# GestaltCogTeam/STEP

Hardware: AMD Instinct MI355X
Metric: training windows/sec on PEMS04, horizon-12 MAE parity, 1/2/4/8 MI355X (higher is better)
Workload: dtype f16 (TSFormer Q/K/weights) + bf16 (P, V, GraphWaveNet / graph-learner GEMMs) operands, f32 accumulate

## Files before the change

### include/step_hip.h

```cpp
#ifndef STEP_HIP_H
#define STEP_HIP_H

#include <stdint.h>

#ifdef __cplusplus
extern "C" {
#endif

const char* step_last_error(void);
int step_abi_version(void);

typedef struct StepGemm {
    int M, N, K, batch;
    const void* A; long sam, sak, sab; int a_bf16;
    const void* B; long sbk, sbn, sbb; int b_bf16;
    float* C; long ldc, scn, scb;
    float alpha;
    int accumulate;
    const float* bias; int relu;
    int splitk;
    int a_kblk; long a_kstride;
    int b_kblk; long b_kstride;
    int b_nblk; long b_nstride;
    int c_nblk; long c_nstride;
// ... 8 lines not shown
int step_gemm(const StepGemm* g, void* stream);

#define STEP_ENC_F16 1
#define STEP_ENC_ALWAYS_RESHIFT 2
#define STEP_ENC_RANGE_FLAG 4
#define STEP_ENC_WORKGROUPS(n) (((n) & 0xffff) << 8)
int step_tsformer_encode(const float* series, int S, int L, const void* wpack, long wpack_bytes,
                         int depth, int flags, uint16_t* hidden_bf16, float* hidden_f32, float* last_f32,
                         float* sqnorm_part, float dropout_p, const uint64_t* drop_pool, long pool_words, uint64_t seed,
                         unsigned int* fallback_count, void* stream);
int step_dropout_pool_fill(uint64_t* pool, long words, float dropout_p, uint64_t seed, void* stream);
long step_tsformer_dropout_words(int L, int depth);

int step_pack_long_history(const float* x, int B, int L, int N, int C, int ch, float* out, void* stream);
int step_gather_windows(const float* data, int T, int N, int C, int ch, const long* t0, int B, int L, int H,
                        float* long_series, float* hist, float* fut, void* stream);

long step_knn_workspace_bytes(int B, int N, int F);
int step_knn_graph(const uint16_t* hidden, const float* sqnorm_part, int B, int N, int F, int k_total,
                   float* sim, float* adj, void* work, long work_bytes, void* stream);
int step_topk_mask(const float* sim, int B, int N, int k_total, float* adj, void* work, long work_bytes,
                   void* stream);

typedef struct StepDglParams {
    float *conv1_w, *conv1_b;
    float *conv2_w, *conv2_b;
    float *fc_w, *fc_b;
    float *bn1_w, *bn1_b, *bn1_rm, *bn1_rv;
    float *bn2_w, *bn2_b, *bn2_rm, *bn2_rv;
    float *bn3_w, *bn3_b, *bn3_rm, *bn3_rv;
    float *fc_out_w, *fc_out_b;
    float *fc_cat_w, *fc_cat_b;
    int gemm_bf16;
} StepDglParams;

long step_dgl_global_saved_floats(int N, int T);
long step_dgl_global_work_floats(int N, int T, int backward);
int step_dgl_global_forward(const float* series_nt, int N, int T, const StepDglParams* p, int training,
                            float momentum, float* saved, float* work, float* g, void* stream);
int step_dgl_global_backward(const float* series_nt, int N, int T, const StepDglParams* p, const float* saved,
                             const float* dg, float* work, const StepDglParams* grads, void* stream);
#define STEP_DGL_FRESH_FC_GRAD 16
int step_dgl_global_backward_phase(const float* series_nt, int N, int T, const StepDglParams* p, const float* saved,
                             const float* dg, float* work, const StepDglParams* grads, int phase, void* stream);

typedef struct StepDglShard { int own1; double count1, count2; } StepDglShard;
int step_dgl_global_forward_shard(const float* series_slice, int N, int Ts, const StepDglParams* p, int training, float momentum,
                                  float* saved, float* work, double* sums, float* g, const StepDglShard* shard, int phase,
                                  void* stream);
int step_dgl_global_backward_shard(const float* series_slice, int N, int Ts, const StepDglParams* p, const float* saved,
                                   const float* dg, float* work, const StepDglParams* grads, const StepDglShard* shard, int phase,
                                   void* stream);
long step_dgl_global_offset(int N, int T, int item);

long step_dgl_edges_saved_floats(int B, int N);
long step_dgl_edges_work_floats(int N);
long step_dgl_edges_theta_offset(int N);
int step_dgl_edges_forward(const float* g, int N, int B, const StepDglParams* p, const float* u, uint64_t seed,
                           float temperature, float* saved, float* theta_out, float* adj_out, void* stream);
int step_dgl_edges_backward(const float* g, int N, int B, const StepDglParams* p, const float* saved,
                            const float* dtheta, const float* dadj, float temperature, float* work,
                            const StepDglParams* grads, float* dg, void* aux_stream, void* stream);

typedef struct StepGwnetParams {
    float *nodevec1, *nodevec2;
    float *start_w, *start_b;
    float *filter_w[8], *filter_b[8];
    float *gate_w[8], *gate_b[8];
    float *skip_w[8], *skip_b[8];
    float *bn_w[8], *bn_b[8], *bn_rm[8], *bn_rv[8];
    float *gconv_w[8], *gconv_b[8];
    float *fc_his0_w, *fc_his0_b, *fc_his2_w, *fc_his2_b;
    float *end1_w, *end1_b, *end2_w, *end2_b;
    int gemm_bf16;
} StepGwnetParams;

long step_gwnet_saved_floats(int B, int N, int dropout);
long step_gwnet_work_floats(int B, int N, int backward);
long step_gwnet_saved_offset(int B, int N, int dropout, int item, int layer);
int step_gwnet_forward(const float* hist, int B, int N, int Cin, const float* hidden_last, const float* adj,
                       const StepGwnetParams* p, int training, float dropout_p, uint64_t seed, float momentum,
                       float* saved, float* work, float* pred, void* stream);
int step_gwnet_forward_phase(const float* hist, int B, int N, int Cin, const float* hidden_last, const float* adj,
                             const StepGwnetParams* p, int training, float dropout_p, uint64_t seed, float momentum,
                             float* saved, float* work, float* pred, int phase, void* stream);
int step_gwnet_backward(const float* hist, int B, int N, int Cin, const float* hidden_last, const StepGwnetParams* p,
                        const float* saved, float* work, const float* dpred, const StepGwnetParams* grads,
                        float* dadj, int dropout, void* aux_stream, void* leaf_stream, void* stream);

int step_pt_dropout(const float* x, float* y, long n, float p, uint64_t seed, uint32_t site, void* stream);
int step_pt_ffn_hidden_fwd(const float* x, const float* w1, const float* b1, long R, float p, uint64_t seed, uint32_t site,
                           uint16_t* hidden, void* stream);
int step_pt_ffn_hidden_bwd(const float* dy, const float* w2, const uint16_t* hidden, long R, float p, uint16_t* dhidden, void* stream);
int step_pt_colsum_bf16(const uint16_t* x, long rows, int cols, float* out, void* stream);
long step_pt_rows_linear_pack_bytes(int nkc, int nog);
int step_pt_rows_linear_pack(const float* w, long swo, long swi, int nkc, int nog, const float* bias, void* pack, void* stream);
int step_pt_rows_linear(const void* x, int x_bf16, long R, const void* pack, int nkc, int nog, void* y, int y_bf16, int accumulate, void* stream);
int step_pt_layer_pack(const float* wi, const float* bi, const float* wo, const float* bo, const float* w1, const float* b1, const float* w2,
                       const float* b2, void* ffn, void* qkv, void* o, void* da, void* dx, void* stream);
long step_pt_proj_wgrad_ws_floats(long R);
int step_pt_proj_wgrad(const float* x, const uint16_t* dqkv, const float* dov, const uint16_t* a, long R, float* ws, float* dwi, float* dbi, float* dwo,
                       void* stream);
int step_pt_ffn_fused_fwd_ln(const float* h1, long R, const void* pack, float p, const uint64_t* pool, long pool_words, uint64_t seed, uint32_t site_hidden,
                             uint32_t site_out, const float* gamma, const float* beta, float* pre, float* y, float* stats, void* stream);
int step_pt_rows_linear_ln(const uint16_t* x, long R, const void* pack, const float* res, float p, uint64_t seed, uint32_t site, const float* gamma,
                           const float* beta, float* pre, float* y, float* stats, void* stream);
// ... 123 lines not shown
```

### step_amd/_lib.py

```python
import ctypes
import os

import torch

_HERE = os.path.dirname(os.path.abspath(__file__))
LIB_PATH = os.environ.get("STEP_HIP_LIB") or os.path.join(_HERE, "libstep_hip.so")

_vp, _i, _l, _f, _u64 = ctypes.c_void_p, ctypes.c_int, ctypes.c_long, ctypes.c_float, ctypes.c_uint64


class StepGemm(ctypes.Structure):
    _fields_ = [("M", _i), ("N", _i), ("K", _i), ("batch", _i),
                ("A", _vp), ("sam", _l), ("sak", _l), ("sab", _l), ("a_bf16", _i),
                ("B", _vp), ("sbk", _l), ("sbn", _l), ("sbb", _l), ("b_bf16", _i),
                ("C", _vp), ("ldc", _l), ("scn", _l), ("scb", _l),
                ("alpha", _f), ("accumulate", _i), ("bias", _vp), ("relu", _i), ("splitk", _i),
                ("a_kblk", _i), ("a_kstride", _l), ("b_kblk", _i), ("b_kstride", _l),
                ("b_nblk", _i), ("b_nstride", _l), ("c_nblk", _i), ("c_nstride", _l),
                ("a_kscale", _vp), ("a_kshift", _vp), ("a_kperiod", _i),
                ("batch0", _i), ("sab1", _l), ("sbb1", _l), ("scb1", _l), ("compute_bf16", _i), ("a_rowsum", _vp), ("c_nscale", _vp), ("c_nshift", _vp), ("c_mvec", _vp),
                ("c_nperiod", _i), ("splitk_ws", _vp), ("splitk_ws_floats", _l)]


class StepDglParams(ctypes.Structure):
    NAMES = ["conv1_w", "conv1_b", "conv2_w", "conv2_b", "fc_w", "fc_b",
             "bn1_w", "bn1_b", "bn1_rm", "bn1_rv", "bn2_w", "bn2_b", "bn2_rm", "bn2_rv",
             "bn3_w", "bn3_b", "bn3_rm", "bn3_rv", "fc_out_w", "fc_out_b", "fc_cat_w", "fc_cat_b"]
    _fields_ = [(n, _vp) for n in NAMES] + [("gemm_bf16", _i)]


class StepGwnetParams(ctypes.Structure):
    _fields_ = [("nodevec1", _vp), ("nodevec2", _vp), ("start_w", _vp), ("start_b", _vp),
                ("filter_w", _vp * 8), ("filter_b", _vp * 8), ("gate_w", _vp * 8), ("gate_b", _vp * 8),
                ("skip_w", _vp * 8), ("skip_b", _vp * 8),
                ("bn_w", _vp * 8), ("bn_b", _vp * 8), ("bn_rm", _vp * 8), ("bn_rv", _vp * 8),
                ("gconv_w", _vp * 8), ("gconv_b", _vp * 8),
                ("fc_his0_w", _vp), ("fc_his0_b", _vp), ("fc_his2_w", _vp), ("fc_his2_b", _vp),
                ("end1_w", _vp), ("end1_b", _vp), ("end2_w", _vp), ("end2_b", _vp), ("gemm_bf16", _i)]


_PD = ctypes.POINTER(StepDglParams)


class StepDynState(ctypes.Structure):
    _fields_ = [("seed_xor", ctypes.c_uint64), ("adam_step", ctypes.c_int32), ("lr", _f), ("gsl_coef", _f), ("reserved", _f)]


class StepDglShard(ctypes.Structure):
    _fields_ = [("own1", ctypes.c_int), ("count1", ctypes.c_double), ("count2", ctypes.c_double)]


_PS = ctypes.POINTER(StepDglShard)
_PG = ctypes.POINTER(StepGwnetParams)

_SIGS = {
    "step_last_error": (ctypes.c_char_p, []),
    "step_abi_version": (_i, []),
    "step_gemm": (_i, [ctypes.POINTER(StepGemm), _vp]),
    "step_tsformer_encode": (_i, [_vp, _i, _i, _vp, _l, _i, _i, _vp, _vp, _vp, _vp, _f, _vp, _l, _u64, _vp, _vp]),
    "step_dropout_pool_fill": (_i, [_vp, _l, _f, _u64, _vp]),
    "step_tsformer_dropout_words": (_l, [_i, _i]),
    "step_gather_windows": (_i, [_vp, _i, _i, _i, _i, _vp, _i, _i, _i, _vp, _vp, _vp, _vp]),
    "step_pack_long_history": (_i, [_vp, _i, _i, _i, _i, _i, _vp, _vp]),
    "step_knn_workspace_bytes": (_l, [_i, _i, _i]),
    "step_knn_graph": (_i, [_vp, _vp, _i, _i, _i, _i, _vp, _vp, _vp, _l, _vp]),
    "step_topk_mask": (_i, [_vp, _i, _i, _i, _vp, _vp, _l, _vp]),
    "step_selftest_mfma": (_i, [_vp, _vp]),
    "step_streams_concurrent": (_i, [_vp, _vp, ctypes.POINTER(_i)]),
    "step_dgl_global_saved_floats": (_l, [_i, _i]),
    "step_dgl_global_work_floats": (_l, [_i, _i, _i]),
    "step_dgl_global_forward": (_i, [_vp, _i, _i, _PD, _i, _f, _vp, _vp, _vp, _vp]),
    "step_dgl_global_backward": (_i, [_vp, _i, _i, _PD, _vp, _vp, _vp, _PD, _vp]),
    "step_dgl_global_backward_phase": (_i, [_vp, _i, _i, _PD, _vp, _vp, _vp, _PD, _i, _vp]),
    "step_dgl_global_forward_shard": (_i, [_vp, _i, _i, _PD, _i, _f, _vp, _vp, _vp, _vp, _PS, _i, _vp]),
    "step_dgl_global_backward_shard": (_i, [_vp, _i, _i, _PD, _vp, _vp, _vp, _PD, _PS, _i, _vp]),
    "step_dgl_global_offset": (_l, [_i, _i, _i]),
    "step_dgl_edges_saved_floats": (_l, [_i, _i]),
    "step_dgl_edges_work_floats": (_l, [_i]),
    "step_dgl_edges_theta_offset": (_l, [_i]),
    "step_dgl_edges_forward": (_i, [_vp, _i, _i, _PD, _vp, _u64, _f, _vp, _vp, _vp, _vp]),
    "step_dgl_edges_backward": (_i, [_vp, _i, _i, _PD, _vp, _vp, _vp, _f, _vp, _PD, _vp, _vp, _vp]),
    "step_gwnet_saved_floats": (_l, [_i, _i, _i]),
    "step_gwnet_work_floats": (_l, [_i, _i, _i]),
    "step_gwnet_saved_offset": (_l, [_i, _i, _i, _i, _i]),
    "step_gwnet_forward": (_i, [_vp, _i, _i, _i, _vp, _vp, _PG, _i, _f, _u64, _f, _vp, _vp, _vp, _vp]),
    "step_gwnet_forward_phase": (_i, [_vp, _i, _i, _i, _vp, _vp, _PG, _i, _f, _u64, _f, _vp, _vp, _vp, _i, _vp]),
    "step_gwnet_backward": (_i, [_vp, _i, _i, _i, _vp, _PG, _vp, _vp, _vp, _PG, _vp, _i, _vp, _vp, _vp]),
    "step_pt_dropout": (_i, [_vp, _vp, _l, _f, _u64, ctypes.c_uint32, _vp]),
    "step_pt_ffn_hidden_fwd": (_i, [_vp, _vp, _vp, _l, _f, _u64, ctypes.c_uint32, _vp, _vp]),
    "step_pt_ffn_hidden_bwd": (_i, [_vp, _vp, _vp, _l, _f, _vp, _vp]),
    "step_pt_colsum_bf16": (_i, [_vp, _l, _i, _vp, _vp]),
    "step_pt_rows_linear_pack_bytes": (_l, [_i, _i]),
    "step_pt_rows_linear_pack": (_i, [_vp, _l, _l, _i, _i, _vp, _vp, _vp]),
    "step_pt_rows_linear": (_i, [_vp, _i, _l, _vp, _i, _i, _vp, _i, _i, _vp]),
    "step_pt_layer_pack": (_i, [_vp] * 14),
    "step_pt_proj_wgrad_ws_floats": (_l, [_l]),
    "step_pt_proj_wgrad": (_i, [_vp, _vp, _vp, _vp, _l, _vp, _vp, _vp, _vp, _vp]),
    "step_pt_ffn_fused_fwd_ln": (_i, [_vp, _l, _vp, _f, _vp, _l, _u64, ctypes.c_uint32, ctypes.c_uint32, _vp, _vp, _vp, _vp, _vp, _vp]),
    "step_pt_rows_linear_ln": (_i, [_vp, _l, _vp, _vp, _f, _u64, ctypes.c_uint32, _vp, _vp, _vp, _vp, _vp, _vp]),
    "step_pt_embed_unmasked_fwd": (_i, [_vp, _vp, _vp, _vp, _vp, _l, _i, _i, _f, _u64, ctypes.c_uint32, _vp, _vp]),
    "step_pt_embed_unmasked_bwd": (_i, [_vp, _vp, _vp, _l, _i, _i, _f, _u64, ctypes.c_uint32, _vp, _vp, _vp, _vp]),
    "step_pt_dec_input_bwd_sums": (_i, [_vp, _l, _i, _i, _f, _u64, ctypes.c_uint32, _vp, _vp, _vp, _vp, _vp]),
    "step_pt_ffn_pack_bytes": (_l, []),
    "step_pt_ffn_wgrad_workgroups": (_l, [_l]),
    "step_pt_ffn_wgrad_ws_floats": (_l, [_l]),
    "step_pt_ffn_pack": (_i, [_vp, _vp, _vp, _vp, _vp, _vp]),
    "step_pt_ffn_fused_fwd": (_i, [_vp, _l, _vp, _f, _vp, _l, _u64, ctypes.c_uint32, _vp, _vp]),
    "step_pt_ffn_fused_bwd_data": (_i, [_vp, _vp, _l, _vp, _f, _vp, _l, _u64, ctypes.c_uint32, _vp, _vp]),
    "step_pt_ffn_fused_bwd_weights": (_i, [_vp, _vp, _l, _vp, _vp, _f, _vp, _l, _u64, ctypes.c_uint32, _vp, _vp, _vp, _vp, _vp]),
    "step_pt_add_layernorm_fwd": (_i, [_vp, _vp, _l, _f, _u64, ctypes.c_uint32, _vp, _vp, _vp, _vp, _vp, _vp]),
    "step_pt_layernorm_bwd_dropout": (_i, [_vp, _vp, _l, _vp, _vp, _vp, _vp, _f, _u64, ctypes.c_uint32, _vp, _vp, _vp, _vp]),
    "step_pt_dropout_relu_mask": (_i, [_vp, _vp, _l, _f, _u64, ctypes.c_uint32, _vp]),
    "step_pt_add_dropout": (_i, [_vp, _vp, _vp, _l, _f, _u64, ctypes.c_uint32, _vp]),
    "step_pt_add_rows": (_i, [_vp, _l, _i, _vp, _vp, _vp]),
    "step_pt_sum_over_seq": (_i, [_vp, _l, _i, _i, _i, _vp, _vp, _vp]),
    "step_pt_token_gather": (_i, [_vp, _l, _i, _vp, _i, _f, _vp, _vp]),
    "step_pt_token_scatter": (_i, [_vp, _l, _i, _vp, _i, _f, _vp, _vp]),
    "step_pt_dec_input": (_i, [_vp, _vp, _vp, _vp, _l, _i, _i, _f, _u64, ctypes.c_uint32, _vp, _vp]),
    "step_pt_dec_input_bwd": (_i, [_vp, _l, _i, _i, _f, _u64, ctypes.c_uint32, _vp, _vp, _vp]),
    "step_pt_layernorm_fwd": (_i, [_vp, _l, _vp, _vp, _vp, _vp, _vp]),
    "step_pt_layernorm_bwd": (_i, [_vp, _vp, _l, _vp, _vp, _vp, _vp, _vp, _vp]),
    "step_pt_attention_fwd": (_i, [_vp, _l, _i, _f, _u64, ctypes.c_uint32, _vp, _vp, _vp]),
    "step_pt_attention_bwd": (_i, [_vp, _vp, _vp, _vp, _l, _i, _f, _u64, ctypes.c_uint32, _vp, _vp]),
    "step_pt_attention_fwd_bf16": (_i, [_vp, _l, _i, _f, _u64, ctypes.c_uint32, _vp, _vp, _vp, _vp, _l, _vp]),
    "step_pt_attention_bwd_bf16": (_i, [_vp, _vp, _vp, _vp, _l, _i, _f, _u64, ctypes.c_uint32, _vp, _vp, _vp]),
    "step_pt_linear_bf16out": (_i, [_vp, _vp, _l, _l, _vp, _l, _i, _i, _vp, _vp]),
    "step_pt_relu_mask": (_i, [_vp, _vp, _l, _vp]),
    "step_colsum": (_i, [_vp, _l, _i, _l, _vp, _vp]),
    "step_loss_fwd_bwd": (_i, [_vp, _vp, _l, _vp, _vp, _l, _f, _f, _vp, _vp, _vp, _vp, _vp]),
# ... 115 lines not shown
```

### step_amd/build.py

```python
import os
import subprocess
import sys

HERE = os.path.dirname(os.path.abspath(__file__))
CSRC = os.path.join(HERE, "csrc")
LIB = os.path.join(HERE, "libstep_hip.so")
SOURCES = ["errors.cpp", "comm.cpp", "gemm.hip", "gemm_bf16.hip", "tsformer_encoder.hip", "knn.hip", "selftest.hip",
           "dgl.hip", "dgl_conv_mfma.hip", "gwnet.hip", "optim.hip", "pretrain.hip", "pretrain_fused.hip", "pretrain_attn2.hip",
           "eval_cache.hip", "eval_metrics.hip", "train_tail.hip"]


def _newer(target, deps):
    if not os.path.exists(target):
        return True
    t = os.path.getmtime(target)
    return any(os.path.getmtime(d) > t for d in deps)


def build(force=False, verbose=True):
    hipcc = os.environ.get("HIPCC", "/opt/rocm/bin/hipcc")
    srcs = [os.path.join(CSRC, s) for s in SOURCES if os.path.exists(os.path.join(CSRC, s))]
    hdrs = [os.path.join(CSRC, f) for f in os.listdir(CSRC) if f.endswith(".h")]
    hdrs.append(os.path.join(HERE, "..", "include", "step_hip.h"))
    objs = []
    os.makedirs(os.path.join(HERE, "build"), exist_ok=True)
    procs = []
    for s in srcs:
        o = os.path.join(HERE, "build", os.path.basename(s) + ".o")
        objs.append(o)
        if force or _newer(o, [s] + hdrs):
            cmd = [hipcc, "--offload-arch=gfx950", "-O3", "-std=c++17", "-fPIC", "-x", "hip", "-c", s, "-o", o]
            if verbose:
                print(" ".join(cmd), flush=True)
            procs.append((s, subprocess.Popen(cmd, stdout=subprocess.PIPE, stderr=subprocess.STDOUT)))
    for s, p in procs:
        out, _ = p.communicate()
        if p.returncode != 0:
            sys.stderr.write(out.decode())
            raise RuntimeError("hipcc failed on " + s)
    if force or _newer(LIB, objs):
        cmd = [hipcc, "--offload-arch=gfx950", "-shared", "-fPIC", "-o", LIB] + objs + ["-ldl"]
        if verbose:
            print(" ".join(cmd), flush=True)
        subprocess.check_call(cmd)
    return LIB


if __name__ == "__main__":
    build(force="--force" in sys.argv)
```

### step_amd/csrc/dgl.hip

```cpp
#include "common.h"
#include "step_internal.h"

namespace {

constexpr int KW = 10;
constexpr int EMB = 100;

template <int CI, int CO, int TPT>
__global__ __launch_bounds__(256) void conv_relu_fwd_kernel(const float* __restrict__ in, const float* __restrict__ w,
                                                            const float* __restrict__ b, const float* __restrict__ in_sc,
                                                            const float* __restrict__ in_sh, float* __restrict__ out,
                                                            float* __restrict__ partial, int Tin, int stat_limit) {
    __shared__ __attribute__((aligned(16))) float ws[CI * KW * CO];
    __shared__ float red[4][2 * CO];
    const int tid = threadIdx.x, n = blockIdx.y;
    const int Tout = Tin - (KW - 1);
    for (int e = tid; e < CI * KW * CO; e += 256) {
        int co = e % CO, k = (e / CO) % KW, ci = e / (CO * KW);
        ws[e] = w[(co * CI + ci) * KW + k];
    }
    __syncthreads();
    const int t0 = (blockIdx.x * 256 + tid) * TPT;
    float acc[CO][TPT];
#pragma unroll
// ... 622 lines not shown
    __shared__ float red[4][32];
    const int o = blockIdx.y, t = blockIdx.x * 256 + threadIdx.x, tid = threadIdx.x;
    const float cso = colsum[o];
    float d[32];
#pragma unroll
    for (int i = 0; i < 32; ++i) d[i] = 0.f;
    if (t < T2) {
        const float4* src = (const float4*)(graw + ((long)o * T2 + t) * 16);
        const float4 g0 = src[0], g1 = src[1], g2 = src[2], g3 = src[3];
        const float g[16] = {g0.x, g0.y, g0.z, g0.w, g1.x, g1.y, g1.z, g1.w, g2.x, g2.y, g2.z, g2.w, g3.x, g3.y, g3.z, g3.w};
        float w[16], old[16];
#pragma unroll
        for (int c = 0; c < 16; ++c) { const long idx = ((long)o * 16 + c) * T2 + t; w[c] = fc_w[idx]; old[c] = overwrite ? 0.f : dfc_w[idx]; }
#pragma unroll
        for (int c = 0; c < 16; ++c) {
            dfc_w[((long)o * 16 + c) * T2 + t] = old[c] + st2[c] * g[c] + st2[16 + c] * cso;
            d[2 * c] = w[c] * g[c]; d[2 * c + 1] = w[c] * cso;
        }
    }
#pragma unroll
    for (int i = 0; i < 32; ++i) {
        const float v = wave_sum(d[i]);
        if ((tid & 63) == 0) red[tid >> 6][i] = v;
    }
    __syncthreads();
    if (tid < 32) atomicAdd(&dots_o[o * 32 + tid], red[0][tid] + red[1][tid] + red[2][tid] + red[3][tid]);
}
__global__ void dots_reduce_kernel(const float* __restrict__ dots_o, float* __restrict__ dots) {
    const int i = threadIdx.x;
    if (i >= 32) return;
    double a = 0.0;
    for (int o = 0; o < EMB; ++o) a += dots_o[o * 32 + i];
    dots[i] = (float)a;
}

static bool dgl_channels_last(const StepDglParams* p) {
    const char* e = getenv("STEP_DGL_F32_STORAGE");
    return p->gemm_bf16 && !(e && e[0] == '1');
}

static bool dgl_legacy_bn_backward() {
    const char* e = getenv("STEP_DGL_LEGACY_BN");
    return e && e[0] == '1';
}

extern "C" long step_dgl_global_saved_floats(int N, int T) {
    long T1 = T - 9, T2 = T - 18;
    return (long)N * 8 * T1 + (long)N * 16 * T2 + (long)N * EMB + 4 * 8 + 4 * 16 + 4 * EMB + (long)EMB * 16 * T2 + 128;
}
static long fc_splitk_ws_floats(int N, int T2) {
    const int splits = step_gemm_auto_splitk(N, EMB, 16 * T2, 1);
    return splits > 1 ? (long)splits * N * EMB + 4 : 0;
}
extern "C" long step_dgl_global_work_floats(int N, int T, int backward) {
    long T1 = T - 9, T2 = T - 18;
    long nb1 = (long)N * cdiv(T1, 1024), nb2 = (long)N * cdiv(T2, 1024);
    long part = (nb1 > nb2 ? nb1 : nb2) * 32 + 64;
    if (!backward) return part + dgl_conv2_pack_floats() + 64 + fc_splitk_ws_floats(N, (int)T2);
    return part + (long)N * 16 * T2 + (long)N * 8 * T1 + (long)EMB * 16 * T2 + 2L * N * EMB + DGL_SMALL + dgl_conv2_wgrad_scratch_floats(N, (int)T1);
}

static float* saved_wp(float* saved, int N, int T) {
    long T1 = T - 9, T2 = T - 18;
    return saved + (long)N * 8 * T1 + (long)N * 16 * T2 + (long)N * EMB + 4 * 8 + 4 * 16 + 4 * EMB;
}
static void carve_saved(float* saved, int N, int T, float** a1, float** a2, float** gpre, float** st1, float** st2, float** st3) {
    long T1 = T - 9, T2 = T - 18;
    *a1 = saved; saved += (long)N * 8 * T1;
    *a2 = saved; saved += (long)N * 16 * T2;
    *gpre = saved; saved += (long)N * EMB;
    *st1 = saved; saved += 4 * 8;
    *st2 = saved; saved += 4 * 16;
    *st3 = saved;
}

static int dgl_bn_stats(const float* partial, int nblk, int C, double count, const float* gamma, const float* beta, float* rm, float* rv,
                        int training, float momentum, float* stat, double* sums, hipStream_t st) {
    if (nblk < 8192) {
        bn_finalize_kernel<<<C, 256, 0, st>>>(partial, nblk, C, count, gamma, beta, rm, rv, training, momentum, stat);
    } else {
        if (hipMemsetAsync(sums, 0, 2 * C * sizeof(double), st) != hipSuccess) { step_set_error("memset failed"); return STEP_ERR_HIP; }
        bn_sums_sliced_kernel<<<dim3(C, 32), 256, 0, st>>>(partial, nblk, C, sums);
        bn_finalize_sums_kernel<<<1, 64, 0, st>>>(sums, C, count, gamma, beta, rm, rv, training, momentum, stat);
    }
    STEP_LAUNCH_CHECK("bn_stats");
    return STEP_OK;
}

static int dgl_global_forward_impl(const float* series_nt, int N, int T, const StepDglParams* p, int training, float momentum,
                                   float* saved, float* work, double* sums, float* g, const StepDglShard* shard, int phase,
                                   hipStream_t st) {
    const int T1 = T - 9, T2 = T - 18;
    float *a1, *a2, *gpre, *st1, *st2, *st3;
    carve_saved(saved, N, T, &a1, &a2, &gpre, &st1, &st2, &st3);
    float* partial = work;
    const bool all = phase == 0;
    const double count1 = shard ? shard->count1 : (double)N * T1, count2 = shard ? shard->count2 : (double)N * T2;
    const bool cl = dgl_channels_last(p);
    const long part_floats = ((long)N * cdiv(T1, 1024) > (long)N * cdiv(T2, 1024) ? (long)N * cdiv(T1, 1024) : (long)N * cdiv(T2, 1024)) * 32 + 64;
    double* own_sums = (double*)(work + part_floats + dgl_conv2_pack_floats());
    float* wp = saved_wp(saved, N, T);
    float* shiftdot = wp + (long)EMB * 16 * T2;
    if (all || phase == 1) {
        int nblk;
        if (cl) {
            STEP_TRY(dgl_conv1_fwd_cl(series_nt, p->conv1_w, p->conv1_b, a1, partial, N, T, shard ? shard->own1 : T1, &nblk, st));
        } else {
            dim3 grid(cdiv(T1, 256 * 4), N);
            conv_relu_fwd_kernel<1, 8, 4><<<grid, 256, 0, st>>>(series_nt, p->conv1_w, p->conv1_b, nullptr, nullptr, a1, partial, T,
                                                                shard ? shard->own1 : T1);
            STEP_LAUNCH_CHECK("conv1");
            nblk = grid.x * grid.y;
        }
        if (shard) bn_sums_kernel<<<8, 256, 0, st>>>(partial, nblk, 8, sums);
        else STEP_TRY(dgl_bn_stats(partial, nblk, 8, count1, p->bn1_w, p->bn1_b, p->bn1_rm, p->bn1_rv, training, momentum, st1, own_sums, st));
        STEP_LAUNCH_CHECK("bn1");
    }
    if (all || phase == 2) {
        if (shard) bn_finalize_sums_kernel<<<1, 64, 0, st>>>(sums, 8, count1, p->bn1_w, p->bn1_b, p->bn1_rm, p->bn1_rv, training, momentum, st1);
        int nblk;
        if (cl) {
            STEP_TRY(dgl_conv2_fwd_cl(a1, p->conv2_w, p->conv2_b, st1, st1 + 8, a2, partial, N, T1, &nblk,
                                      work + part_floats, st));
        } else if (p->gemm_bf16) {
            STEP_TRY(dgl_conv2_fwd_mfma(a1, p->conv2_w, p->conv2_b, st1, st1 + 8, a2, partial, N, T1, &nblk, st));
        } else {
            dim3 grid(cdiv(T2, 256 * 4), N);
            conv_relu_fwd_kernel<8, 16, 4><<<grid, 256, 0, st>>>(a1, p->conv2_w, p->conv2_b, st1, st1 + 8, a2, partial, T1, T2);
            STEP_LAUNCH_CHECK("conv2");
            nblk = grid.x * grid.y;
        }
        if (shard) bn_sums_kernel<<<16, 256, 0, st>>>(partial, nblk, 16, sums + 16);
        else STEP_TRY(dgl_bn_stats(partial, nblk, 16, count2, p->bn2_w, p->bn2_b, p->bn2_rm, p->bn2_rv, training, momentum, st2, own_sums, st));
        STEP_LAUNCH_CHECK("bn2");
    }
    if (all || phase == 3) {
        if (shard) bn_finalize_sums_kernel<<<1, 64, 0, st>>>(sums + 16, 16, count2, p->bn2_w, p->bn2_b, p->bn2_rm, p->bn2_rv, training, momentum, st2);
        const long K = 16L * T2;
        StepGemm gm = gemm_desc(N, EMB, (int)K, a2, K, 1, p->fc_w, 1, K, gpre, EMB);
        if (cl) {
            if (hipMemsetAsync(shiftdot, 0, 128 * sizeof(float), st) != hipSuccess) { step_set_error("memset failed"); return STEP_ERR_HIP; }
            fc_prep_kernel<<<dim3(cdiv(T2, 256), EMB), 256, 0, st>>>(p->fc_w, st2, (uint4*)wp, shiftdot, T2);
            gpre_init_kernel<<<cdiv((long)N * EMB, 256), 256, 0, st>>>(gpre, shiftdot, (long)N * EMB);
            STEP_LAUNCH_CHECK("fc_prep");
            gm.a_bf16 = 1;
            gm.B = wp; gm.b_bf16 = 1;
        } else {
            if (hipMemsetAsync(gpre, 0, (size_t)N * EMB * sizeof(float), st) != hipSuccess) { step_set_error("memset failed"); return STEP_ERR_HIP; }
            gm.a_kscale = st2; gm.a_kshift = st2 + 16; gm.a_kperiod = T2;
        }
        gm.accumulate = 2;
        gm.splitk = -1;
        gm.compute_bf16 = p->gemm_bf16;
        if (fc_splitk_ws_floats(N, T2) > 0) {
            float* ws = work + part_floats + dgl_conv2_pack_floats() + 64;
            gm.splitk_ws = (float*)(((uintptr_t)ws + 15) & ~(uintptr_t)15);
            gm.splitk_ws_floats = fc_splitk_ws_floats(N, T2) - 4;
        }
        STEP_TRY(step_gemm_launch(gm, st));
    }
    if (all || phase == 4) {
        fc_post_bn3_kernel<<<EMB, 256, 0, st>>>(gpre, p->fc_b, N, p->bn3_w, p->bn3_b, p->bn3_rm, p->bn3_rv, training, momentum, st3, g);
        STEP_LAUNCH_CHECK("fc_post_bn3");
    }
    return STEP_OK;
}

extern "C" int step_dgl_global_forward(const float* series_nt, int N, int T, const StepDglParams* p, int training,
                                       float momentum, float* saved, float* work, float* g, void* stream) {
    STEP_REQUIRE(series_nt && p && saved && work && g && N > 0 && T > 18, "dgl_global_forward: bad arguments");
    return dgl_global_forward_impl(series_nt, N, T, p, training, momentum, saved, work, nullptr, g, nullptr, 0, (hipStream_t)stream);
}

extern "C" int step_dgl_global_forward_shard(const float* series_slice, int N, int Ts, const StepDglParams* p, int training,
                                             float momentum, float* saved, float* work, double* sums, float* g,
                                             const StepDglShard* shard, int phase, void* stream) {
    STEP_REQUIRE(series_slice && p && saved && work && sums && g && shard && N > 0 && Ts > 18 && phase >= 1 && phase <= 4,
                 "dgl_global_forward_shard: bad arguments");
    STEP_REQUIRE(shard->own1 > 0 && shard->own1 <= Ts - 9 && shard->count1 > 0 && shard->count2 > 0, "dgl_global_forward_shard: bad shard");
    return dgl_global_forward_impl(series_slice, N, Ts, p, training, momentum, saved, work, sums, g, shard, phase, (hipStream_t)stream);
}

extern "C" long step_dgl_global_offset(int N, int T, int item) {
    const long T1 = T - 9, T2 = T - 18;
    if (item == 0) return 0;
    if (item == 1) return (long)N * 8 * T1;
    if (item == 2) return (long)N * 8 * T1 + (long)N * 16 * T2;
    const long nb1 = (long)N * cdiv(T1, 1024), nb2 = (long)N * cdiv(T2, 1024);
    const long coef = (nb1 > nb2 ? nb1 : nb2) * 32 + 64 + (long)N * 16 * T2 + (long)N * 8 * T1 + (long)EMB * 16 * T2 + 2L * N * EMB;
    if (item == 10) return coef + 256;
    if (item == 11) return coef + 320;
    return -1;
}

static int dgl_global_backward_impl(const float* series_nt, int N, int T, const StepDglParams* p, const float* saved, const float* dg,
                                    float* work, const StepDglParams* grads, const StepDglShard* shard, int phase, void* stream);

extern "C" int step_dgl_global_backward(const float* series_nt, int N, int T, const StepDglParams* p, const float* saved,
                                        const float* dg, float* work, const StepDglParams* grads, void* stream) {
    return step_dgl_global_backward_phase(series_nt, N, T, p, saved, dg, work, grads, 0, stream);
}

extern "C" int step_dgl_global_backward_phase(const float* series_nt, int N, int T, const StepDglParams* p, const float* saved,
                                              const float* dg, float* work, const StepDglParams* grads, int phase, void* stream) {
    STEP_REQUIRE(series_nt && p && saved && dg && work && grads && N > 0 && T > 18 && (phase & ~STEP_DGL_FRESH_FC_GRAD) >= 0 &&
                 (phase & ~STEP_DGL_FRESH_FC_GRAD) <= 2, "dgl_global_backward: bad arguments");
    return dgl_global_backward_impl(series_nt, N, T, p, saved, dg, work, grads, nullptr, phase, stream);
}

extern "C" int step_dgl_global_backward_shard(const float* series_slice, int N, int Ts, const StepDglParams* p, const float* saved,
                                              const float* dg, float* work, const StepDglParams* grads, const StepDglShard* shard,
                                              int phase, void* stream) {
    const int ph = phase & ~STEP_DGL_FRESH_FC_GRAD;
    STEP_REQUIRE(series_slice && p && saved && dg && work && grads && shard && N > 0 && Ts > 18 && (ph == 1 || ph == 3 || ph == 4),
                 "dgl_global_backward_shard: bad arguments");
    STEP_REQUIRE(p->gemm_bf16 && Ts - 18 >= 128, "dgl_global_backward_shard: needs the bf16 contraction mode and a slice of >= 128 conv2 columns");
    return dgl_global_backward_impl(series_slice, N, Ts, p, saved, dg, work, grads, shard, phase, stream);
}

static int dgl_global_backward_impl(const float* series_nt, int N, int T, const StepDglParams* p, const float* saved, const float* dg,
                                    float* work, const StepDglParams* grads, const StepDglShard* shard, int phase, void* stream) {
    const int fresh_fc = (phase & STEP_DGL_FRESH_FC_GRAD) ? 1 : 0;
    phase &= ~STEP_DGL_FRESH_FC_GRAD;
    const bool do_fc = phase == 0 || phase == 1, do_mid = phase == 0 || phase == 2 || phase == 3, do_tail = phase == 0 || phase == 2 || phase == 4;
    hipStream_t st = (hipStream_t)stream;
    const int T1 = T - 9, T2 = T - 18;
    const long K = 16L * T2;
    float *a1, *a2, *gpre, *st1, *st2, *st3;
    carve_saved((float*)saved, N, T, &a1, &a2, &gpre, &st1, &st2, &st3);
    long nb1 = (long)N * cdiv(T1, 1024), nb2 = (long)N * cdiv(T2, 1024);
    float* partial = work;
    float* d_a2 = work + (nb1 > nb2 ? nb1 : nb2) * 32 + 64;
    float* d_a1 = d_a2 + (long)N * 16 * T2;
    float* wraw = d_a1 + (long)N * 8 * T1;
    float* dgpre = wraw + (long)EMB * K;
    float* dgpreT = dgpre + (long)N * EMB;
    float* coef = dgpreT + (long)N * EMB;
    float* dots = coef + 256;
    float* graw = coef + 320;
    float* wg_scratch = coef + DGL_SMALL;
// ... 195 lines not shown
```

### step_amd/csrc/step_internal.h

```cpp
#pragma once
#include <hip/hip_runtime.h>
#include <vector>
#include "../../include/step_hip.h"

enum { GEMM_FUSED_INTERLEAVED = 1, GEMM_FUSED_FFN_FWD = 2, GEMM_FUSED_MASKNZ = 4, GEMM_FUSED_BF16OUT = 8 };
struct GemmFused {
    const float* dotw; float* dots;
    const float* bnx; const float* bncoef; const float* bnstat;
    int channels, period;
    int flags;
    const float* ffn_bias; const void* maskx; float p; unsigned seed_lo, seed_hi, site;
};

struct GemmKSeg { long a_off, b_off, a_bs, b_bs; int a_rs, b_rs; };
constexpr int GEMM_KSEG_MAX = 128;
int step_gemm_segmented_launch(StepGemm g, const GemmKSeg* ktab, int ktab_per, hipStream_t st);

int step_gemm_launch(StepGemm g, hipStream_t st);
int step_gemm_auto_splitk(int M, int N, int K, int batch);
int step_gemm_launch_fused(StepGemm g, const GemmFused& fused, hipStream_t st);
int step_gemm_bf16_launch(StepGemm g, hipStream_t st, const GemmFused* fused = nullptr);
int step_gemm_f32_fast_launch(StepGemm g, hipStream_t st, const GemmFused* fused = nullptr);

static inline StepGemm gemm_desc(int M, int N, int K, const float* A, long sam, long sak, const float* B, long sbk,
                                 long sbn, float* C, long ldc) {
    StepGemm g;
    memset(&g, 0, sizeof(g));
    g.M = M; g.N = N; g.K = K; g.batch = 1;
    g.A = A; g.sam = sam; g.sak = sak;
    g.B = B; g.sbk = sbk; g.sbn = sbn;
    g.C = C; g.ldc = ldc; g.scn = 1;
    g.alpha = 1.f; g.splitk = 1;
    return g;
}

int step_gemm_rowsum_separate(StepGemm* g, hipStream_t st);
int dgl_conv2_fwd_mfma(const float* a1, const float* w, const float* b, const float* sc, const float* sh, float* a2, float* partial,
                       int N, int T1, int* nblk, hipStream_t st);
int dgl_conv2_dgrad_mfma(const float* dz, const float* w, float* din, int N, int T1, const float* bnx, const float* coef, const float* stat,
                         int own, hipStream_t st);
int dgl_conv2_wgrad_xhat_mfma(const float* dz, const float* a1, const float* stat1, float* scratch, float* graw, int N, int T1, hipStream_t st);
int dgl_conv2_wgrad_finish(const float* graw, const float* w, const float* stat1, const float* gamma1, const float* beta1, double count,
                           float* dw, float* db, float* dgamma1, float* dbeta1, float* coef1, int raw, hipStream_t st);
int dgl_conv1_fwd_cl(const float* x, const float* w, const float* b, void* a1h, float* partial, int N, int T, int stat_limit, int* nblk,
                     hipStream_t st);
long dgl_conv2_pack_floats();
int dgl_conv2_fwd_cl(const void* a1h, const float* w, const float* b, const float* sc, const float* sh, void* a2h, float* partial, int N,
                     int T1, int* nblk, float* pack, hipStream_t st);
int dgl_conv2_dgrad_cl(const void* dz2h, const float* w, const float* sc, void* dz1h, int N, int T1, const void* a1h, const float* coef,
                       const float* stat, int own, float* pack, hipStream_t st);
int dgl_conv2_wgrad_cl(const void* dz2h, const void* a1h, float* scratch, float* graw, int N, int T1, hipStream_t st);
int dgl_conv1_wgrad_cl(const void* dz1h, const float* x, float* scratch, float* dw, float* db, int N, int T, hipStream_t st);
long dgl_conv2_wgrad_scratch_floats(int N, int T1);
int dgl_conv2_wgrad_mfma(const float* dz, const float* a1, const float* sc, const float* sh, float* scratch, float* dw, float* db, int N,
                         int T1, hipStream_t st);
int dgl_conv1_wgrad_mfma(const float* dz, const float* x, float* scratch, float* dw, float* db, int N, int T, hipStream_t st);
int step_colsum_launch(const float* x, long rows, int cols, long ld, float* out, hipStream_t st);

struct AuxLane {
    hipStream_t main, aux;
    bool on;
    int next = 0, base = 0;
    AuxLane(hipStream_t m, hipStream_t a, int base_ = 0) : main(m), aux(a), on(a != nullptr && a != m), base(base_) {}
    static hipEvent_t event(int k) {
        thread_local std::vector<hipEvent_t> pool[16];
        int dev = 0;
        (void)hipGetDevice(&dev);
        std::vector<hipEvent_t>& v = pool[dev & 15];
        while ((int)v.size() <= k) {
            hipEvent_t e;
            if (hipEventCreateWithFlags(&e, hipEventDisableTiming) != hipSuccess) return nullptr;
            v.push_back(e);
        }
        return v[k];
    }
    hipStream_t fork() {
        if (!on) return main;
        hipEvent_t e = event(base + (next++ & 63));
        if (!e || hipEventRecord(e, main) != hipSuccess || hipStreamWaitEvent(aux, e, 0) != hipSuccess) { on = false; return main; }
        return aux;
    }
    hipEvent_t mark() {
        if (!on) return nullptr;
        hipEvent_t e = event(base + (next++ & 63));
        if (!e || hipEventRecord(e, main) != hipSuccess) { on = false; return nullptr; }
        return e;
    }
    hipStream_t after(hipEvent_t e) {
        if (!on || !e) return main;
        if (hipStreamWaitEvent(aux, e, 0) != hipSuccess) { on = false; return main; }
        return aux;
    }
    hipEvent_t done() {
        if (!on) return nullptr;
        hipEvent_t e = event(base + (next++ & 63));
        if (!e || hipEventRecord(e, aux) != hipSuccess) return nullptr;
        return e;
    }
    int wait_done(hipEvent_t e) {
// ... 16 lines not shown
```

Before: 2364.

## Add streaming fused fc forward kernel for the DGL global graph learner

Measured after the change: 2356. No clear change (-0.3%).

```diff
diff --git a/include/step_hip.h b/include/step_hip.h
--- a/include/step_hip.h
+++ b/include/step_hip.h
@@ -84,6 +84,7 @@
                                    const float* dg, float* work, const StepDglParams* grads, const StepDglShard* shard, int phase,
                                    void* stream);
 long step_dgl_global_offset(int N, int T, int item);
+long step_dgl_fc_stream_plan(int N, int T2, int* out);
 
 long step_dgl_edges_saved_floats(int B, int N);
 long step_dgl_edges_work_floats(int N);
diff --git a/step_amd/_lib.py b/step_amd/_lib.py
--- a/step_amd/_lib.py
+++ b/step_amd/_lib.py
@@ -75,6 +75,7 @@
     "step_dgl_global_forward_shard": (_i, [_vp, _i, _i, _PD, _i, _f, _vp, _vp, _vp, _vp, _PS, _i, _vp]),
     "step_dgl_global_backward_shard": (_i, [_vp, _i, _i, _PD, _vp, _vp, _vp, _PD, _PS, _i, _vp]),
     "step_dgl_global_offset": (_l, [_i, _i, _i]),
+    "step_dgl_fc_stream_plan": (_l, [_i, _i, ctypes.POINTER(ctypes.c_int)]),
     "step_dgl_edges_saved_floats": (_l, [_i, _i]),
     "step_dgl_edges_work_floats": (_l, [_i]),
     "step_dgl_edges_theta_offset": (_l, [_i]),
diff --git a/step_amd/build.py b/step_amd/build.py
--- a/step_amd/build.py
+++ b/step_amd/build.py
@@ -6,7 +6,7 @@
 CSRC = os.path.join(HERE, "csrc")
 LIB = os.path.join(HERE, "libstep_hip.so")
 SOURCES = ["errors.cpp", "comm.cpp", "gemm.hip", "gemm_bf16.hip", "tsformer_encoder.hip", "knn.hip", "selftest.hip",
-           "dgl.hip", "dgl_conv_mfma.hip", "gwnet.hip", "optim.hip", "pretrain.hip", "pretrain_fused.hip", "pretrain_attn2.hip",
+           "dgl.hip", "dgl_fc_stream.hip", "dgl_fc_stream_plan.cpp", "dgl_conv_mfma.hip", "gwnet.hip", "optim.hip", "pretrain.hip", "pretrain_fused.hip", "pretrain_attn2.hip",
            "eval_cache.hip", "eval_metrics.hip", "train_tail.hip"]
 
 
diff --git a/step_amd/csrc/dgl.hip b/step_amd/csrc/dgl.hip
--- a/step_amd/csrc/dgl.hip
+++ b/step_amd/csrc/dgl.hip
@@ -698,11 +698,23 @@
     const int splits = step_gemm_auto_splitk(N, EMB, 16 * T2, 1);
     return splits > 1 ? (long)splits * N * EMB + 4 : 0;
 }
+static long fc_ws_floats(int N, int T2) {
+    int pl[6];
+    const long a = fc_splitk_ws_floats(N, T2), b = step_dgl_fc_stream_plan(N, T2, pl) + 4;
+    return a > b ? a : b;
+}
+static int dgl_fc_stream_mode(int N, int T2) {
+    const char* e = getenv("STEP_DGL_FC_STREAM");
+    if (!e || !e[0]) return N <= 320 && T2 < DGL_FC_STREAM_MAX_T2 ? 1 : 0;
+    if (!strcmp(e, "0")) return 0;
+    if (!strcmp(e, "1") || !strcmp(e, "fwd")) return 1;
+    return -1;
+}
 extern "C" long step_dgl_global_work_floats(int N, int T, int backward) {
     long T1 = T - 9, T2 = T - 18;
     long nb1 = (long)N * cdiv(T1, 1024), nb2 = (long)N * cdiv(T2, 1024);
     long part = (nb1 > nb2 ? nb1 : nb2) * 32 + 64;
-    if (!backward) return part + dgl_conv2_pack_floats() + 64 + fc_splitk_ws_floats(N, (int)T2);
+    if (!backward) return part + dgl_conv2_pack_floats() + 64 + fc_ws_floats(N, (int)T2);
     return part + (long)N * 16 * T2 + (long)N * 8 * T1 + (long)EMB * 16 * T2 + 2L * N * EMB + DGL_SMALL + dgl_conv2_wgrad_scratch_floats(N, (int)T1);
 }
 
@@ -783,27 +795,34 @@
     if (all || phase == 3) {
         if (shard) bn_finalize_sums_kernel<<<1, 64, 0, st>>>(sums + 16, 16, count2, p->bn2_w, p->bn2_b, p->bn2_rm, p->bn2_rv, training, momentum, st2);
         const long K = 16L * T2;
-        StepGemm gm = gemm_desc(N, EMB, (int)K, a2, K, 1, p->fc_w, 1, K, gpre, EMB);
-        if (cl) {
-            if (hipMemsetAsync(shiftdot, 0, 128 * sizeof(float), st) != hipSuccess) { step_set_error("memset failed"); return STEP_ERR_HIP; }
-            fc_prep_kernel<<<dim3(cdiv(T2, 256), EMB), 256, 0, st>>>(p->fc_w, st2, (uint4*)wp, shiftdot, T2);
-            gpre_init_kernel<<<cdiv((long)N * EMB, 256), 256, 0, st>>>(gpre, shiftdot, (long)N * EMB);
-            STEP_LAUNCH_CHECK("fc_prep");
-            gm.a_bf16 = 1;
-            gm.B = wp; gm.b_bf16 = 1;
+        float* ws = work + part_floats + dgl_conv2_pack_floats() + 64;
+        ws = (float*)(((uintptr_t)ws + 15) & ~(uintptr_t)15);
+        const int stream_mode = cl ? dgl_fc_stream_mode(N, T2) : 0;
+        STEP_REQUIRE(stream_mode >= 0, "dgl_global_forward: STEP_DGL_FC_STREAM must be 0, 1 or fwd");
+        if (stream_mode == 1) {
+            STEP_TRY(dgl_fc_fwd_stream(a2, p->fc_w, st2, wp, shiftdot, ws, gpre, N, T2, st));
         } else {
-            if (hipMemsetAsync(gpre, 0, (size_t)N * EMB * sizeof(float), st) != hipSuccess) { step_set_error("memset failed"); return STEP_ERR_HIP; }
-            gm.a_kscale = st2; gm.a_kshift = st2 + 16; gm.a_kperiod = T2;
-        }
-        gm.accumulate = 2;
-        gm.splitk = -1;
-        gm.compute_bf16 = p->gemm_bf16;
-        if (fc_splitk_ws_floats(N, T2) > 0) {
-            float* ws = work + part_floats + dgl_conv2_pack_floats() + 64;
-            gm.splitk_ws = (float*)(((uintptr_t)ws + 15) & ~(uintptr_t)15);
-            gm.splitk_ws_floats = fc_splitk_ws_floats(N, T2) - 4;
-        }
-        STEP_TRY(step_gemm_launch(gm, st));
+            StepGemm gm = gemm_desc(N, EMB, (int)K, a2, K, 1, p->fc_w, 1, K, gpre, EMB);
+            if (cl) {
+                if (hipMemsetAsync(shiftdot, 0, 128 * sizeof(float), st) != hipSuccess) { step_set_error("memset failed"); return STEP_ERR_HIP; }
+                fc_prep_kernel<<<dim3(cdiv(T2, 256), EMB), 256, 0, st>>>(p->fc_w, st2, (uint4*)wp, shiftdot, T2);
+                gpre_init_kernel<<<cdiv((long)N * EMB, 256), 256, 0, st>>>(gpre, shiftdot, (long)N * EMB);
+                STEP_LAUNCH_CHECK("fc_prep");
+                gm.a_bf16 = 1;
+                gm.B = wp; gm.b_bf16 = 1;
+            } else {
+                if (hipMemsetAsync(gpre, 0, (size_t)N * EMB * sizeof(float), st) != hipSuccess) { step_set_error("memset failed"); return STEP_ERR_HIP; }
+                gm.a_kscale = st2; gm.a_kshift = st2 + 16; gm.a_kperiod = T2;
+            }
+            gm.accumulate = 2;
+            gm.splitk = -1;
+            gm.compute_bf16 = p->gemm_bf16;
+            if (fc_splitk_ws_floats(N, T2) > 0) {
+                gm.splitk_ws = ws;
+                gm.splitk_ws_floats = fc_splitk_ws_floats(N, T2) - 4;
+            }
+            STEP_TRY(step_gemm_launch(gm, st));
+        }
     }
     if (all || phase == 4) {
         fc_post_bn3_kernel<<<EMB, 256, 0, st>>>(gpre, p->fc_b, N, p->bn3_w, p->bn3_b, p->bn3_rm, p->bn3_rv, training, momentum, st3, g);
@@ -832,6 +851,7 @@
     if (item == 0) return 0;
     if (item == 1) return (long)N * 8 * T1;
     if (item == 2) return (long)N * 8 * T1 + (long)N * 16 * T2;
+    if (item == 3) return (long)N * 8 * T1 + (long)N * 16 * T2 + (long)N * EMB + 4 * 8 + 4 * 16 + 4 * EMB;
     const long nb1 = (long)N * cdiv(T1, 1024), nb2 = (long)N * cdiv(T2, 1024);
     const long coef = (nb1 > nb2 ? nb1 : nb2) * 32 + 64 + (long)N * 16 * T2 + (long)N * 8 * T1 + (long)EMB * 16 * T2 + 2L * N * EMB;
     if (item == 10) return coef + 256;
diff --git a/step_amd/csrc/dgl_fc_stream.hip b/step_amd/csrc/dgl_fc_stream.hip
--- /dev/null
+++ b/step_amd/csrc/dgl_fc_stream.hip
@@ -0,0 +1,207 @@
+#include "common.h"
+#include "step_internal.h"
+
+extern "C" long step_dgl_fc_stream_plan(int N, int T2, int* out);
+
+namespace {
+
+constexpr int FS_EMB = 100;
+constexpr int FS_CHUNK = 16;
+constexpr int FS_SLAB_BYTES = 320 * 128;
+constexpr int FS_WROW = FS_CHUNK * 32 + 16;
+constexpr int FS_WBYTES = FS_EMB * FS_WROW;
+constexpr int FS_LDS = 2 * FS_SLAB_BYTES + FS_WBYTES + 128 + 512;
+constexpr int FS_UNITS = 14;
+
+__device__ __forceinline__ void fs_dma_1k(const char* base, uint32_t off, uint32_t lds_dst) {
+    uint32_t keep;
+    lds_dst = __builtin_amdgcn_readfirstlane(lds_dst);
+    asm volatile("s_mov_b32 %0, m0\n\ts_mov_b32 m0, %3\n\ts_nop 0\n\tglobal_load_lds_dwordx4 %1, %2\n\ts_mov_b32 m0, %0"
+                 : "=&s"(keep)
+                 : "v"(off), "s"(base), "s"(lds_dst)
+                 : "memory");
+}
+
+#define FS_W(x) w##x##0, w##x##1, w##x##2, w##x##3, w##x##4, w##x##5, w##x##6, w##x##7, w##x##8, w##x##9, w##x##10, w##x##11, w##x##12, w##x##13
+#define FS_LD(m) wload(m, lane_off, wa##m, wb##m);
+#define FS_CV(m) conv(m, wa##m, wb##m);
+
+__global__ __launch_bounds__(1024) void fc_fwd_stream_kernel(const char* __restrict__ a2h, const float* __restrict__ fc_w,
+                                                             const float* __restrict__ st2, char* __restrict__ wp, float* __restrict__ part,
+                                                             float* __restrict__ shiftpart, int N, int T2, int rows, int cps, int nch) {
+    extern __shared__ __attribute__((aligned(16))) char fs_lds[];
+    char* wl = fs_lds + 2 * FS_SLAB_BYTES;
+    float* stl = (float*)(wl + FS_WBYTES);
+    const int tid = threadIdx.x, lane = tid & 63, wave = __builtin_amdgcn_readfirstlane(tid >> 6);
+    const int s = blockIdx.x, rb = blockIdx.y, S = gridDim.x;
+    const int row0 = rb * rows, nrt = rows >> 5;
+    const int ch0 = s * cps;
+    const int nchunk = min(cps, nch - ch0);
+    const int ct = wave & 3, rg = wave >> 2;
+    const int tl = lane & 15, cq = lane >> 4;
+    float* shl = stl + 32;
+    if (tid < 32) stl[tid] = st2[tid];
+    if (lane < 8) shl[wave + 16 * lane] = 0.f;
+    f32x16 acc[3];
+#pragma unroll
+    for (int i = 0; i < 3; ++i)
+#pragma unroll
+        for (int e = 0; e < 16; ++e) acc[i][e] = 0.f;
+    const uint32_t lds0 = (uint32_t)(uintptr_t)(__attribute__((address_space(3))) char*)fs_lds;
+    const char* a2b = a2h + (long)row0 * T2 * 32;
+    const int pc = (lane & 7) ^ (lane >> 3);
+    uint32_t rowoff[3];
+#pragma unroll
+    for (int i = 0; i < 3; ++i) rowoff[i] = (uint32_t)(min(row0 + (wave + 16 * i) * 8 + (lane >> 3), N - 1) - row0) * (uint32_t)T2 * 32u + (pc & 1) * 16;
+    auto issue = [&](int ts, int buf) {
+        const uint32_t toff = (uint32_t)min(ts + (pc >> 1), T2 - 1) * 32u;
+#pragma unroll
+        for (int i = 0; i < 3; ++i) {
+            const int g = wave + 16 * i;
+            if (g < nrt * 4) fs_dma_1k(a2b, rowoff[i] + toff, lds0 + (uint32_t)(buf * FS_SLAB_BYTES + g * 1024));
+        }
+    };
+    float FS_W(a), FS_W(b);
+    auto wload = [&](int m, uint32_t lane_off, float& a, float& b) {
+        const int o = min(wave + 16 * (m >> 1), FS_EMB - 1);
+        const char* base = (const char*)(fc_w + ((long)o * 16 + 8 * (m & 1)) * T2);
+        a = *(const float*)(base + lane_off);
+        b = *(const float*)(base + (lane_off + 4u * (uint32_t)T2));
+    };
+    {
+        const uint32_t lane_off = 4u * (uint32_t)(2 * cq * T2 + min(ch0 * FS_CHUNK + tl, T2 - 1));
+        FS_LD(0) FS_LD(1) FS_LD(2) FS_LD(3) FS_LD(4) FS_LD(5) FS_LD(6) FS_LD(7) FS_LD(8) FS_LD(9) FS_LD(10) FS_LD(11) FS_LD(12) FS_LD(13)
+    }
+    issue(ch0 * FS_CHUNK, 0);
+    for (int q = 0; q < nchunk; ++q) {
+        const int t0 = (ch0 + q) * FS_CHUNK;
+        const bool more = q + 1 < nchunk;
+#pragma unroll
+        for (int j = 0; j < 4; ++j) {
+            asm volatile("s_waitcnt vmcnt(0)" ::: "memory");
+            if (j == 0) {
+                __syncthreads();
+                int lc = lane;
+                asm volatile("" : "+v"(lc));
+                const int tl = lc & 15, cq = lc >> 4;
+                const float live = t0 + tl < T2 ? 1.f : 0.f;
+                float sh = 0.f, mine = 0.f;
+                auto conv = [&](int m, float wa, float wb) {
+                    const int jo = m >> 1, o = wave + 16 * jo, c2 = cq + 4 * (m & 1);
+                    if (jo < 6 || o < FS_EMB) {
+                        const float w0 = wa * live, w1 = wb * live;
+                        sh += w0 * stl[16 + 2 * c2] + w1 * stl[17 + 2 * c2];
+                        *(uint32_t*)(wl + o * FS_WROW + tl * 32 + c2 * 4) = pack_bf16x2(w0 * stl[2 * c2], w1 * stl[2 * c2 + 1]);
+                        if (m & 1) {
+                            sh = wave_sum(sh);
+                            mine = lane == jo ? sh : mine;
+                            sh = 0.f;
+                        }
+                    }
+                };
+                FS_CV(0) FS_CV(1) FS_CV(2) FS_CV(3) FS_CV(4) FS_CV(5) FS_CV(6) FS_CV(7) FS_CV(8) FS_CV(9) FS_CV(10) FS_CV(11) FS_CV(12) FS_CV(13)
+                if (lane < FS_UNITS / 2 && wave + 16 * lane < FS_EMB) shl[wave + 16 * lane] += mine;
+            }
+            __syncthreads();
+            if (j < 3 || more) issue(t0 + (j + 1) * 4, (j + 1) & 1);
+            if (more) {
+                const uint32_t lane_off = 4u * (uint32_t)(2 * cq * T2 + min(t0 + FS_CHUNK + tl, T2 - 1));
+                if (j == 0) { FS_LD(0) FS_LD(1) FS_LD(2) FS_LD(3) }
+                if (j == 1) { FS_LD(4) FS_LD(5) FS_LD(6) FS_LD(7) }
+                if (j == 2) { FS_LD(8) FS_LD(9) FS_LD(10) }
+                if (j == 3) { FS_LD(11) FS_LD(12) FS_LD(13) }
+            }
+            if (j == 0 && rb == 0) {
+#pragma unroll
+                for (int i = 0; i < 4; ++i) {
+                    int tt = tid;
+                    asm volatile("" : "+v"(tt));
+                    const int o = (tt >> 5) + 32 * i, piece = tt & 31;
+                    char* base = wp + ((long)32 * i * T2 + t0) * 32;
+                    if (o < FS_EMB && t0 + (piece >> 1) < T2)
+                        *(uint4*)(base + ((uint32_t)(tt >> 5) * (uint32_t)T2 * 32u + piece * 16)) = *(const uint4*)(wl + o * FS_WROW + piece * 16);
+                }
+            }
+            const char* slab = fs_lds + (j & 1) * FS_SLAB_BYTES;
+            int ln = lane;
+            asm volatile("" : "+v"(ln));
+            const int r = ln & 31, h = ln >> 5;
+            const int ob = min(ct * 32 + r, FS_EMB - 1);
+#pragma unroll
+            for (int ks = 0; ks < 4; ++ks) {
+                __builtin_amdgcn_sched_barrier(0);
+                const bf16x8 b = *(const bf16x8*)(wl + ob * FS_WROW + (j * 4 + ks) * 32 + h * 16);
+                const int sl = ((ks * 2 + h) ^ (r & 7)) << 4;
+#pragma unroll
+                for (int i = 0; i < 3; ++i) {
+                    const int rt = rg + 4 * i;
+                    if (rt < nrt) {
+                        const bf16x8 a = *(const bf16x8*)(slab + (rt * 32 + r) * 128 + sl);
+                        acc[i] = __builtin_amdgcn_mfma_f32_32x32x16_bf16(a, b, acc[i], 0, 0, 0);
+                    }
+                }
+            }
+        }
+    }
+    if (rb == 0 && lane < FS_UNITS / 2 && wave + 16 * lane < FS_EMB) shiftpart[s * 128 + wave + 16 * lane] = shl[wave + 16 * lane];
+#pragma unroll
+    for (int i = 0; i < 3; ++i) {
+        const int rt = rg + 4 * i;
+        if (rt < nrt) {
+            float* o = part + (((long)rb * S + s) * (nrt * 4) + rt * 4 + ct) * 1024 + lane;
+#pragma unroll
+            for (int e = 0; e < 16; ++e) o[e * 64] = acc[i][e];
+        }
+    }
+}
+
+__global__ __launch_bounds__(256) void fc_fwd_stream_reduce_kernel(const float* __restrict__ part, const float* __restrict__ shiftpart, int S, int NT,
+                                                                    int rows, int N, float* __restrict__ gpre, float* __restrict__ shiftdot) {
+    __shared__ float sh[32];
+    const int rb = blockIdx.x / NT, tile = blockIdx.x % NT, rt = tile >> 2, ct = tile & 3;
+    const int tid = threadIdx.x, lane = tid & 63, eg = tid >> 6;
+    if (tid < 32) {
+        const int o = ct * 32 + tid;
+        float v = 0.f;
+        if (o < FS_EMB)
+            for (int s = 0; s < S; ++s) v += shiftpart[s * 128 + o];
+        sh[tid] = v;
+        if (o < FS_EMB && blockIdx.x == (unsigned)ct) shiftdot[o] = v;
+    }
+    __syncthreads();
+    const long sstr = (long)NT * 1024;
+    const int col = ct * 32 + (lane & 31);
+#pragma unroll
+    for (int ee = 0; ee < 4; ++ee) {
+        const int e = eg * 4 + ee;
+        const float* src = part + ((long)rb * S * NT + tile) * 1024 + e * 64 + lane;
+        float v0 = 0.f, v1 = 0.f, v2 = 0.f, v3 = 0.f;
+        int sp = 0;
+        for (; sp + 4 <= S; sp += 4) {
+            v0 += src[(long)sp * sstr]; v1 += src[(long)(sp + 1) * sstr]; v2 += src[(long)(sp + 2) * sstr]; v3 += src[(long)(sp + 3) * sstr];
+        }
+        for (; sp < S; ++sp) v0 += src[(long)sp * sstr];
+        const int row = rb * rows + rt * 32 + 8 * (e >> 2) + (e & 3) + 4 * (lane >> 5);
+        if (row < N && col < FS_EMB) gpre[(long)row * FS_EMB + col] = ((v0 + v1) + (v2 + v3)) + sh[lane & 31];
+    }
+}
+
+}
+
+int dgl_fc_fwd_stream(const void* a2h, const float* fc_w, const float* st2, void* wp, float* shiftdot, float* ws, float* gpre, int N, int T2,
+                      hipStream_t st) {
+    int pl[6];
+    const long floats = step_dgl_fc_stream_plan(N, T2, pl);
+    STEP_REQUIRE(floats > 0 && pl[2] == FS_CHUNK && pl[4] <= 320, "fc_fwd_stream: bad plan");
+    STEP_REQUIRE(T2 < DGL_FC_STREAM_MAX_T2, "fc_fwd_stream: more than %d time steps (32-bit row offsets)", DGL_FC_STREAM_MAX_T2 - 1);
+    const int RB = pl[0], S = pl[1], cps = pl[3], rows = pl[4], NT = pl[5];
+    STEP_TRY(step_raise_lds_once((const void*)fc_fwd_stream_kernel, FS_LDS, "fc_fwd_stream"));
+    float* part = ws;
+    float* shiftpart = ws + (long)RB * S * NT * 1024;
+    fc_fwd_stream_kernel<<<dim3(S, RB), 1024, FS_LDS, st>>>((const char*)a2h, fc_w, st2, (char*)wp, part, shiftpart, N, T2, rows, cps,
+                                                            cdiv(T2, FS_CHUNK));
+    STEP_LAUNCH_CHECK("fc_fwd_stream");
+    fc_fwd_stream_reduce_kernel<<<RB * NT, 256, 0, st>>>(part, shiftpart, S, NT, rows, N, gpre, shiftdot);
+    STEP_LAUNCH_CHECK("fc_fwd_stream_reduce");
+    return STEP_OK;
+}
diff --git a/step_amd/csrc/dgl_fc_stream_plan.cpp b/step_amd/csrc/dgl_fc_stream_plan.cpp
--- /dev/null
+++ b/step_amd/csrc/dgl_fc_stream_plan.cpp
@@ -0,0 +1,27 @@
+#include <stdint.h>
+
+extern "C" long step_dgl_fc_stream_plan(int N, int T2, int* out);
+
+namespace {
+constexpr int kMaxRows = 320, kChunk = 16, kTargetGroups = 96;
+}
+
+extern "C" long step_dgl_fc_stream_plan(int N, int T2, int* out) {
+    if (N < 1 || T2 < 1 || !out) return 0;
+    const int rb = (int)(((long)N + kMaxRows - 1) / kMaxRows);
+    const int rows = (int)(((((long)N + rb - 1) / rb) + 31) / 32 * 32);
+    const int nch = (int)(((long)T2 + kChunk - 1) / kChunk);
+    int want = kTargetGroups / rb;
+    if (want < 1) want = 1;
+    if (want > nch) want = nch;
+    const int cps = (nch + want - 1) / want;
+    const int slices = (nch + cps - 1) / cps;
+    const int tiles = rows / 32 * 4;
+    out[0] = rb;
+    out[1] = slices;
+    out[2] = kChunk;
+    out[3] = cps;
+    out[4] = rows;
+    out[5] = tiles;
+    return (long)rb * slices * tiles * 1024 + (long)slices * 128;
+}
diff --git a/step_amd/csrc/step_internal.h b/step_amd/csrc/step_internal.h
--- a/step_amd/csrc/step_internal.h
+++ b/step_amd/csrc/step_internal.h
@@ -45,6 +45,9 @@
 int dgl_conv1_fwd_cl(const float* x, const float* w, const float* b, void* a1h, float* partial, int N, int T, int stat_limit, int* nblk,
                      hipStream_t st);
 long dgl_conv2_pack_floats();
+constexpr int DGL_FC_STREAM_MAX_T2 = 400000;
+int dgl_fc_fwd_stream(const void* a2h, const float* fc_w, const float* st2, void* wp, float* shiftdot, float* ws, float* gpre, int N, int T2,
+                      hipStream_t st);
 int dgl_conv2_fwd_cl(const void* a1h, const float* w, const float* b, const float* sc, const float* sh, void* a2h, float* partial, int N,
                      int T1, int* nblk, float* pack, hipStream_t st);
 int dgl_conv2_dgrad_cl(const void* dz2h, const float* w, const float* sc, void* dz1h, int N, int T1, const void* a1h, const float* coef,
```
